# ReactiveBayes/Cortex.jl

Hardware: NVIDIA B200
Metric: message_updates_per_sec (higher is better)
Workload: dtype f32

## Files before the change

### cortex.jl_b200/csrc/grid.cu

```cuda
#include <cmath>

#include <cstring>

#include "common.cuh"

namespace cxb {

template <class T, int E>
struct VecE;
template <>
struct VecE<float, 4> {
    using type = float4;
};
template <>
struct VecE<double, 2> {
    using type = double2;
};

template <class T, int E>
__device__ __forceinline__ void load_vec(const T* p, T (&v)[E]) {
    using V = typename VecE<T, E>::type;
    V x = __ldcs(reinterpret_cast<const V*>(p));
    const T* s = reinterpret_cast<const T*>(&x);
#pragma unroll
    for (int k = 0; k < E; ++k) v[k] = s[k];
}
template <class T, int E>
__device__ __forceinline__ void store_vec(T* p, const T (&v)[E]) {
    using V = typename VecE<T, E>::type;
    V x;
    T* s = reinterpret_cast<T*>(&x);
#pragma unroll
    for (int k = 0; k < E; ++k) s[k] = v[k];
    __stcs(reinterpret_cast<V*>(p), x);
}
template <class T, int E, int LP>
__device__ __forceinline__ T group_sum(const T (&v)[E]) {
    T s = v[0];
#pragma unroll
    for (int k = 1; k < E; ++k) s += v[k];
#pragma unroll
    for (int o = LP / 2; o > 0; o >>= 1) s += __shfl_xor_sync(0xffffffffu, s, o, LP);
    return s;
}

template <class T>
__device__ __forceinline__ T rcp_pos(T x) {
    if constexpr (sizeof(T) == 4) {
        float q;
        asm("rcp.approx.ftz.f32 %0, %1;" : "=f"(q) : "f"(x));
        return fmaf(q, fmaf(-x, q, 1.0f), q);
    } else {
        return T(1) / x;
    }
}

template <class T, int E, int LP>
__device__ __forceinline__ void potts_m2v(const T (&in)[E], bool ex, T w, T (&mv)[E], bool store, void* plane, size_t o) {
    const T S = group_sum<T, E, LP>(in);
#pragma unroll
    for (int k = 0; k < E; ++k) mv[k] = S + w * in[k];
    const T tot = group_sum<T, E, LP>(mv);
    if (ex) {
        const T inv = rcp_pos<T>(tot);
#pragma unroll
        for (int k = 0; k < E; ++k) mv[k] = mv[k] * inv;
        if (store) store_vec<T, E>((T*)plane + o, mv);
    } else {
#pragma unroll
        for (int k = 0; k < E; ++k) mv[k] = T(1);
    }
}

struct GridView {
    long long H, W;
    int has_up, has_down;
    int eager_m2v;
    const void* unary;
    const void* m2f_cur[4];
    void* m2f_nxt[4];
    void* m2v[4];
    void* marg;
    const void* halo_up;
    const void* halo_down;
    void* peer_up;
    void* peer_down;
};

template <class T, int K, int E>
__global__ void __launch_bounds__(256) k_potts_sweep(GridView g, T w) {
    constexpr int LP = K / E;
    static_assert(LP >= 1 && LP <= 32 && (LP & (LP - 1)) == 0, "K / E must be a power of two <= 32");
    const long long npix = g.H * g.W;
    const long long gid = (long long)blockIdx.x * blockDim.x + threadIdx.x;
    long long pix = gid / LP;
    const int lane = (int)(gid % LP);
    const bool valid = pix < npix;
    if (!valid) pix = npix - 1;
    const long long i = pix / g.W, j = pix % g.W;
    const size_t o = (size_t)pix * K + (size_t)lane * E;

    bool ex[4];
    ex[0] = i > 0 || g.has_up;
    ex[1] = j > 0;
    ex[2] = j + 1 < g.W;
    ex[3] = i + 1 < g.H || g.has_down;

    T un[E];
    load_vec<T, E>((const T*)g.unary + o, un);

    T in[4][E];
    {
        const T* src[4];
        src[0] = (i > 0) ? (const T*)g.m2f_cur[3] + o - (size_t)g.W * K : (const T*)g.halo_up + (size_t)j * K + (size_t)lane * E;
        src[1] = (const T*)g.m2f_cur[2] + o - K;
        src[2] = (const T*)g.m2f_cur[1] + o + K;
        src[3] = (i + 1 < g.H) ? (const T*)g.m2f_cur[0] + o + (size_t)g.W * K
                               : (const T*)g.halo_down + (size_t)j * K + (size_t)lane * E;
#pragma unroll
        for (int d = 0; d < 4; ++d) {
            if (ex[d]) {
                load_vec<T, E>(src[d], in[d]);
            } else {
#pragma unroll
                for (int k = 0; k < E; ++k) in[d][k] = T(1);
            }
        }
    }
    const bool store_mv = valid && (g.eager_m2v || i == 0 || i + 1 == g.H);
    T mv[4][E];
#pragma unroll
    for (int d = 0; d < 4; ++d) {
        potts_m2v<T, E, LP>(in[d], ex[d], w, mv[d], store_mv, g.m2v[d], o);
    }
    {
        T acc[E];
#pragma unroll
        for (int k = 0; k < E; ++k) {
            T a = un[k];
            if (ex[0]) a = a * mv[0][k];
            if (ex[1]) a = a * mv[1][k];
            if (ex[2]) a = a * mv[2][k];
            if (ex[3]) a = a * mv[3][k];
            acc[k] = a;
        }
        const T inv_tot = rcp_pos<T>(group_sum<T, E, LP>(acc));
#pragma unroll
        for (int k = 0; k < E; ++k) acc[k] = acc[k] * inv_tot;
        if (valid) store_vec<T, E>((T*)g.marg + o, acc);
    }
#pragma unroll
    for (int d = 0; d < 4; ++d) {
        T acc[E];
#pragma unroll
        for (int k = 0; k < E; ++k) {
            T a = un[k];
#pragma unroll
            for (int d2 = 0; d2 < 4; ++d2)
                if (d2 != d && ex[d2]) a = a * mv[d2][k];
            acc[k] = a;
        }
        const T inv_tot = rcp_pos<T>(group_sum<T, E, LP>(acc));
#pragma unroll
        for (int k = 0; k < E; ++k) acc[k] = acc[k] * inv_tot;
        if (valid && ex[d]) store_vec<T, E>((T*)g.m2f_nxt[d] + o, acc);
        if (d == 0 && valid && i == 0 && g.peer_up) store_vec<T, E>((T*)g.peer_up + (size_t)j * K + (size_t)lane * E, acc);
        if (d == 3 && valid && i + 1 == g.H && g.peer_down) store_vec<T, E>((T*)g.peer_down + (size_t)j * K + (size_t)lane * E, acc);
    }
}

template <class T, int K, int E>
__global__ void __launch_bounds__(256) k_potts_m2v(GridView g, T w) {
    constexpr int LP = K / E;
    const long long npix = (g.H - 2) * g.W;
    const long long gid = (long long)blockIdx.x * blockDim.x + threadIdx.x;
    long long q = gid / LP;
    const int lane = (int)(gid % LP);
    const bool valid = q < npix;
    if (!valid) q = npix - 1;
    const long long pix = q + g.W;
    const long long j = pix % g.W;
    const size_t o = (size_t)pix * K + (size_t)lane * E;
    const bool ex[4] = {true, j > 0, j + 1 < g.W, true};
    const T* src[4];
    src[0] = (const T*)g.m2f_cur[3] + o - (size_t)g.W * K;
    src[1] = (const T*)g.m2f_cur[2] + o - K;
    src[2] = (const T*)g.m2f_cur[1] + o + K;
    src[3] = (const T*)g.m2f_cur[0] + o + (size_t)g.W * K;
    T in[4][E];
#pragma unroll
    for (int d = 0; d < 4; ++d) {
        if (ex[d]) {
            load_vec<T, E>(src[d], in[d]);
        } else {
#pragma unroll
            for (int k = 0; k < E; ++k) in[d][k] = T(1);
        }
    }
#pragma unroll
    for (int d = 0; d < 4; ++d) {
        T mv[E];
        potts_m2v<T, E, LP>(in[d], ex[d], w, mv, valid, g.m2v[d], o);
    }
}

__global__ void k_halo_wait(const volatile unsigned* flag_a, const volatile unsigned* flag_b, unsigned expected, unsigned long long timeout_ns,
                            unsigned* timed_out) {
    unsigned long long t0;
    asm volatile("mov.u64 %0, %%globaltimer;" : "=l"(t0));
    auto wait = [&](const volatile unsigned* f, unsigned bit) {
        while (*f < expected) {
            __nanosleep(64);
            unsigned long long t;
            asm volatile("mov.u64 %0, %%globaltimer;" : "=l"(t));
            if (t - t0 > timeout_ns) {
                atomicOr(timed_out, bit);
                return;
            }
        }
    };
    if (flag_a) wait(flag_a, 1u);
    if (flag_b) wait(flag_b, 2u);
    __threadfence_system();
}
__global__ void k_halo_signal(unsigned* peer_flag_a, unsigned* peer_flag_b, unsigned value) {
    __threadfence_system();
    if (peer_flag_a) *(volatile unsigned*)peer_flag_a = value;
    if (peer_flag_b) *(volatile unsigned*)peer_flag_b = value;
    __threadfence_system();
}

template <class T>
__global__ void k_fill(T* p, size_t n, T v) {
    size_t i = (size_t)blockIdx.x * blockDim.x + threadIdx.x;
    if (i < n) p[i] = v;
}

struct Grid {
    int device = 0, dtype = CXB_F32, K = 0, has_up = 0, has_down = 0, cur = 0;
    long long H = 0, W = 0;
    double beta = 0;
    cudaStream_t stream = nullptr;
    cudaEvent_t ev0 = nullptr, ev1 = nullptr;
    std::string err;
    DBuf<unsigned char> unary, m2f[2], m2v, marg, halo_recv;
    DBuf<unsigned> flags;
    DBuf<unsigned char> unary_alt, marg_alt;
    unsigned char *cur_unary = nullptr, *cur_marg = nullptr;
    cudaStream_t s_in = nullptr, s_out = nullptr;
    cudaEvent_t ev_in[2] = {nullptr, nullptr}, ev_sw[2] = {nullptr, nullptr}, ev_out[2] = {nullptr, nullptr};
    unsigned long long job_no = 0;
    unsigned sweep_no = 0;
    unsigned long long halo_timeout_ns = 20ull * 1000000000ull;
    bool eager_m2v = false, m2v_pending = false;
    int32_t check_halo() {
        if (!peer_halo[0] && !peer_halo[1]) return CXB_OK;
        unsigned t = 0;
        if (cudaMemcpy(&t, flags.p + 2, sizeof(unsigned), cudaMemcpyDeviceToHost) != cudaSuccess) return CXB_ERR_CUDA;
        if (!t) return CXB_OK;
        err = std::string("fused halo exchange: the row neighbour ") + ((t & 1) ? "above" : "below") +
              " did not deliver its boundary messages in time (its sweep was never enqueued, or the process is gone)";
        return CXB_ERR_STATE;
    }
    unsigned char* peer_halo[2] = {nullptr, nullptr};
    unsigned* peer_flags[2] = {nullptr, nullptr};
    void* ipc_opened[4] = {nullptr, nullptr, nullptr, nullptr};
    bool have_unary = false, have_msgs = false, ran = false;
    size_t esz() const { return dtype == CXB_F32 ? 4 : 8; }
    size_t plane() const { return (size_t)H * W * K * esz(); }
    size_t row() const { return (size_t)W * K * esz(); }
    ~Grid() {
        for (void* q : ipc_opened)
            if (q) cudaIpcCloseMemHandle(q);
        if (ev0) cudaEventDestroy(ev0);
        if (ev1) cudaEventDestroy(ev1);
        for (int i = 0; i < 2; ++i) {
            if (ev_in[i]) cudaEventDestroy(ev_in[i]);
            if (ev_sw[i]) cudaEventDestroy(ev_sw[i]);
            if (ev_out[i]) cudaEventDestroy(ev_out[i]);
        }
        if (s_in) cudaStreamDestroy(s_in);
        if (s_out) cudaStreamDestroy(s_out);
        if (stream) cudaStreamDestroy(stream);
    }
    int32_t init() {
        int count = 0;
        if (cudaGetDeviceCount(&count) != cudaSuccess || count == 0) {
            err = "no CUDA device available (cortex_b200 has no CPU fallback)";
            return CXB_ERR_CUDA;
        }
        int E = dtype == CXB_F32 ? 4 : 2;
        int LP = K / E;
        if (device < 0 || device >= count || H <= 0 || W <= 0 || K < E || K % E || LP > 32 || (LP & (LP - 1))) {
            err = "bad device / shape (labels must be 4,8,...,128 for fp32 and 2,4,...,64 for fp64, a power of two)";
            return CXB_ERR_BAD_ARG;
        }
        CXB_CUDA(cudaSetDevice(device));
        CXB_CUDA(cudaStreamCreateWithFlags(&stream, cudaStreamNonBlocking));
        if (const char* e = getenv("CXB_GRID_HALO_TIMEOUT_MS")) halo_timeout_ns = (unsigned long long)std::max(1, atoi(e)) * 1000000ull;
        if (const char* e = getenv("CXB_GRID_EAGER_M2V")) eager_m2v = atoi(e) != 0;
        CXB_CUDA(cudaEventCreate(&ev0));
        CXB_CUDA(cudaEventCreate(&ev1));
        CXB_CUDA(unary.reserve(plane()));
        CXB_CUDA(m2f[0].reserve(4 * plane()));
        CXB_CUDA(m2f[1].reserve(4 * plane()));
        CXB_CUDA(m2v.reserve(4 * plane()));
        CXB_CUDA(marg.reserve(plane()));
        CXB_CUDA(halo_recv.reserve(4 * row()));
        CXB_CUDA(flags.reserve(4));
        CXB_CUDA(cudaMemsetAsync(flags.p, 0, 4 * sizeof(unsigned), stream));
        CXB_CUDA(cudaMemsetAsync(m2v.p, 0, 4 * plane(), stream));
        CXB_CUDA(cudaMemsetAsync(marg.p, 0, plane(), stream));
        return CXB_OK;
    }
    template <class T>
    int32_t fill(void* p, size_t n, double v) {
        CXB_LAUNCH(k_fill<T>, cdiv(n, 256), 256, 0, stream, (T*)p, n, (T)v);
        return CXB_OK;
    }
    int32_t reset() {
        CXB_CUDA(cudaSetDevice(device));
        if (int32_t st = flush_m2v()) return st;
        size_t n = (size_t)4 * H * W * K, nh = (size_t)4 * W * K;
        double u = 1.0 / K;
        for (int b = 0; b < 2; ++b) dtype == CXB_F32 ? fill<float>(m2f[b].p, n, u) : fill<double>(m2f[b].p, n, u);
        dtype == CXB_F32 ? fill<float>(halo_recv.p, nh, u) : fill<double>(halo_recv.p, nh, u);
        CXB_CUDA(cudaMemsetAsync(flags.p, 0, 4 * sizeof(unsigned), stream));
        CXB_CUDA(cudaGetLastError());
        CXB_CUDA(cudaStreamSynchronize(stream));
        cur = 0;
        sweep_no = 0;
        have_msgs = true;
        return CXB_OK;
    }
    GridView view(int in) const {
        GridView g{};
        g.H = H;
        g.W = W;
        g.has_up = has_up;
        g.has_down = has_down;
        g.eager_m2v = eager_m2v;
        for (int d = 0; d < 4; ++d) {
            g.m2f_cur[d] = m2f[in].p + (size_t)d * plane();
            g.m2f_nxt[d] = m2f[in ^ 1].p + (size_t)d * plane();
            g.m2v[d] = m2v.p + (size_t)d * plane();
        }
        return g;
    }
    template <class T, int E>
    int32_t launch_k(const GridView& g, bool m2v_only) {
        const T w = (T)(std::exp(beta) - 1.0);
        long long threads = (m2v_only ? H - 2 : H) * W * (K / E);
        unsigned grid = cdiv((size_t)threads, 256);
        switch (K / E) {
#define CASE(LPV)                                                                                      \
    case LPV:                                                                                          \
        if (m2v_only)                                                                                  \
            CXB_LAUNCH((k_potts_m2v<T, LPV * E, E>), grid, 256, 0, stream, g, w);                      \
        else                                                                                           \
            CXB_LAUNCH((k_potts_sweep<T, LPV * E, E>), grid, 256, 0, stream, g, w);                    \
        break;
            CASE(1)
            CASE(2)
            CASE(4)
            CASE(8)
            CASE(16)
            CASE(32)
#undef CASE
        }
        return CXB_OK;
    }
    int32_t sweep(int64_t* n_updates) {
        if (!have_unary || !have_msgs) {
            err = "set the unary evidence and reset the messages first";
            return CXB_ERR_STATE;
        }
        CXB_CUDA(cudaSetDevice(device));
        GridView g = view(cur);
        g.unary = cur_unary ? cur_unary : unary.p;
        g.marg = cur_marg ? cur_marg : marg.p;
        const size_t par = (size_t)(sweep_no & 1) * 2 * row(), nxt_par = (size_t)((sweep_no + 1) & 1) * 2 * row();
        g.halo_up = halo_recv.p + par;
        g.halo_down = halo_recv.p + par + row();
        g.peer_up = peer_halo[0] ? peer_halo[0] + nxt_par + row() : nullptr;
        g.peer_down = peer_halo[1] ? peer_halo[1] + nxt_par : nullptr;
        const bool fused = peer_halo[0] || peer_halo[1];
        if (fused && sweep_no > 0)
            CXB_LAUNCH(k_halo_wait, 1, 1, 0, stream, peer_halo[0] ? flags.p + 0 : nullptr, peer_halo[1] ? flags.p + 1 : nullptr, sweep_no,
                       halo_timeout_ns, flags.p + 2);
        CXB_CUDA(cudaEventRecord(ev0, stream));
        int32_t st = dtype == CXB_F32 ? launch_k<float, 4>(g, false) : launch_k<double, 2>(g, false);
        if (st) return st;
        CXB_CUDA(cudaEventRecord(ev1, stream));
        m2v_pending = !eager_m2v;
        if (fused)
            CXB_LAUNCH(k_halo_signal, 1, 1, 0, stream, peer_flags[0] ? peer_flags[0] + 1 : nullptr, peer_flags[1] ? peer_flags[1] + 0 : nullptr,
                       sweep_no + 1);
        CXB_CUDA(cudaGetLastError());
        cur ^= 1;
        ++sweep_no;
        ran = true;
        if (n_updates) {
            long long vert = (H - 1) * W * 2 + (has_up ? W : 0) + (has_down ? W : 0);
            long long horz = H * (W - 1) * 2;
            *n_updates = 2 * (vert + horz) + H * W;
        }
        return CXB_OK;
    }
    int32_t flush_m2v() {
        if (!m2v_pending) return CXB_OK;
        CXB_CUDA(cudaSetDevice(device));
        if (H > 2) {
            const GridView g = view(cur ^ 1);
            int32_t st = dtype == CXB_F32 ? launch_k<float, 4>(g, true) : launch_k<double, 2>(g, true);
            if (st) return st;
            CXB_CUDA(cudaGetLastError());
        }
        m2v_pending = false;
        return CXB_OK;
    }
    int32_t infer_host(const void* unary_host, void* marg_out_host, int n_sweeps, int64_t* n_updates) {
        if (!have_msgs) {
            err = "reset the messages first";
            return CXB_ERR_STATE;
        }
        CXB_CUDA(cudaSetDevice(device));
        if (!s_in) {
            CXB_CUDA(unary_alt.reserve(plane()));
            CXB_CUDA(marg_alt.reserve(plane()));
            CXB_CUDA(cudaStreamCreateWithFlags(&s_in, cudaStreamNonBlocking));
            CXB_CUDA(cudaStreamCreateWithFlags(&s_out, cudaStreamNonBlocking));
            for (int i = 0; i < 2; ++i) {
                CXB_CUDA(cudaEventCreateWithFlags(&ev_in[i], cudaEventDisableTiming));
                CXB_CUDA(cudaEventCreateWithFlags(&ev_sw[i], cudaEventDisableTiming));
                CXB_CUDA(cudaEventCreateWithFlags(&ev_out[i], cudaEventDisableTiming));
            }
            CXB_CUDA(cudaStreamSynchronize(stream));
        }
        const int b = (int)(job_no & 1);
        unsigned char* U = b ? unary_alt.p : unary.p;
        unsigned char* M = b ? marg_alt.p : marg.p;
        if (job_no >= 2) CXB_CUDA(cudaStreamWaitEvent(s_in, ev_sw[b], 0));
        CXB_CUDA(cudaMemcpyAsync(U, unary_host, plane(), cudaMemcpyHostToDevice, s_in));
        CXB_CUDA(cudaEventRecord(ev_in[b], s_in));
        CXB_CUDA(cudaStreamWaitEvent(stream, ev_in[b], 0));
        if (job_no >= 2) CXB_CUDA(cudaStreamWaitEvent(stream, ev_out[b], 0));
        cur_unary = U;
        cur_marg = M;
        have_unary = true;
        int64_t upd = 0;
        for (int k = 0; k < n_sweeps; ++k) {
            int32_t st = sweep(&upd);
            if (st) return st;
        }
        CXB_CUDA(cudaEventRecord(ev_sw[b], stream));
        CXB_CUDA(cudaStreamWaitEvent(s_out, ev_sw[b], 0));
        CXB_CUDA(cudaMemcpyAsync(marg_out_host, M, plane(), cudaMemcpyDeviceToHost, s_out));
        CXB_CUDA(cudaEventRecord(ev_out[b], s_out));
        ++job_no;
        if (n_updates) *n_updates = upd * n_sweeps;
        return CXB_OK;
    }
    int32_t sync_all() {
        CXB_CUDA(cudaSetDevice(device));
        CXB_CUDA(cudaStreamSynchronize(stream));
        if (s_in) CXB_CUDA(cudaStreamSynchronize(s_in));
        if (s_out) CXB_CUDA(cudaStreamSynchronize(s_out));
        return check_halo();
    }
};

}

using cxb::Grid;
static inline Grid* GR(cxb_grid* g) { return reinterpret_cast<Grid*>(g); }
#define GR_CUDA(g, expr)                                        \
    do {                                                        \
        cudaError_t e__ = (expr);                               \
        if (e__ != cudaSuccess) {                               \
            GR(g)->err = ::cxb::cuda_msg(e__, #expr);           \
            return CXB_ERR_CUDA;                                \
        }                                                       \
    } while (0)

extern "C" {

int32_t cxb_grid_create(int32_t device, int32_t dtype, int64_t rows, int64_t cols, int32_t n_labels, double beta,
                        int32_t has_upper, int32_t has_lower, cxb_grid** out) try {
    if (!out || (dtype != CXB_F32 && dtype != CXB_F64)) return CXB_ERR_BAD_ARG;
    *out = nullptr;
    Grid* g = new Grid();
    g->device = device;
    g->dtype = dtype;
    g->H = rows;
    g->W = cols;
    g->K = n_labels;
    g->beta = beta;
    g->has_up = has_upper ? 1 : 0;
    g->has_down = has_lower ? 1 : 0;
    int32_t st = g->init();
    if (st) {
        fprintf(stderr, "cxb_grid_create: %s\n", g->err.c_str());
        delete g;
        return st;
    }
    *out = reinterpret_cast<cxb_grid*>(g);
    return CXB_OK;
} CXB_ABI_CATCH(CXB_ERR_INTERNAL)
void cxb_grid_destroy(cxb_grid* g) {
    if (g) {
        cudaSetDevice(GR(g)->device);
        delete GR(g);
    }
}
const char* cxb_grid_last_error(cxb_grid* g) { return g ? GR(g)->err.c_str() : "null handle"; }
int32_t cxb_grid_set_unary(cxb_grid* g, const void* unary_host) try {
    Grid* h = GR(g);
    GR_CUDA(g, cudaSetDevice(h->device));
    GR_CUDA(g, cudaMemcpyAsync(h->cur_unary ? h->cur_unary : h->unary.p, unary_host, h->plane(), cudaMemcpyHostToDevice, h->stream));
    GR_CUDA(g, cudaStreamSynchronize(h->stream));
    h->have_unary = true;
    return CXB_OK;
} CXB_ABI_CATCH(CXB_ERR_INTERNAL)
int32_t cxb_grid_reset_messages(cxb_grid* g) try { return GR(g)->reset(); } CXB_ABI_CATCH(CXB_ERR_INTERNAL)
int32_t cxb_grid_sweep(cxb_grid* g, int64_t* n_updates_out) try { return GR(g)->sweep(n_updates_out); } CXB_ABI_CATCH(CXB_ERR_INTERNAL)
void* cxb_grid_halo_send_ptr(cxb_grid* g, int32_t direction) {
    Grid* h = GR(g);
    unsigned char* base = h->m2f[h->cur].p;
    if (direction == 0) return base + 0 * h->plane();
    if (direction == 1) return base + 3 * h->plane() + (size_t)(h->H - 1) * h->row();
    return nullptr;
}
void* cxb_grid_halo_recv_ptr(cxb_grid* g, int32_t direction) {
    Grid* h = GR(g);
    unsigned char* base = h->halo_recv.p + (size_t)(h->sweep_no & 1) * 2 * h->row();
    if (direction == 0) return base;
    if (direction == 1) return base + h->row();
    return nullptr;
}
int32_t cxb_grid_p2p_export(cxb_grid* g, void* handles_out) try {
    Grid* h = GR(g);
    GR_CUDA(g, cudaSetDevice(h->device));
    cudaIpcMemHandle_t hh[2];
    GR_CUDA(g, cudaIpcGetMemHandle(&hh[0], h->halo_recv.p));
    GR_CUDA(g, cudaIpcGetMemHandle(&hh[1], h->flags.p));
    memcpy(handles_out, hh, sizeof(hh));
    return CXB_OK;
} CXB_ABI_CATCH(CXB_ERR_INTERNAL)
int32_t cxb_grid_p2p_connect_ipc(cxb_grid* g, int32_t direction, const void* neighbour_handles) try {
    Grid* h = GR(g);
    if (direction != 0 && direction != 1) return CXB_ERR_BAD_ARG;
    GR_CUDA(g, cudaSetDevice(h->device));
    cudaIpcMemHandle_t hh[2];
    memcpy(hh, neighbour_handles, sizeof(hh));
    void *halo = nullptr, *fl = nullptr;
    GR_CUDA(g, cudaIpcOpenMemHandle(&halo, hh[0], cudaIpcMemLazyEnablePeerAccess));
    GR_CUDA(g, cudaIpcOpenMemHandle(&fl, hh[1], cudaIpcMemLazyEnablePeerAccess));
    h->ipc_opened[2 * direction] = halo;
    h->ipc_opened[2 * direction + 1] = fl;
    h->peer_halo[direction] = (unsigned char*)halo;
    h->peer_flags[direction] = (unsigned*)fl;
    return CXB_OK;
} CXB_ABI_CATCH(CXB_ERR_INTERNAL)
int32_t cxb_grid_p2p_connect_local(cxb_grid* g, int32_t direction, cxb_grid* neighbour) try {
    Grid *h = GR(g), *nb = GR(neighbour);
    if ((direction != 0 && direction != 1) || !nb || nb->W != h->W || nb->K != h->K || nb->dtype != h->dtype) return CXB_ERR_BAD_ARG;
    if (nb->device != h->device) {
        int can = 0;
        GR_CUDA(g, cudaDeviceCanAccessPeer(&can, h->device, nb->device));
        if (!can) {
            h->err = "no peer access between the two devices";
            return CXB_ERR_CUDA;
        }
        GR_CUDA(g, cudaSetDevice(h->device));
        cudaError_t e = cudaDeviceEnablePeerAccess(nb->device, 0);
        if (e != cudaSuccess && e != cudaErrorPeerAccessAlreadyEnabled) GR_CUDA(g, e);
        (void)cudaGetLastError();
    }
    h->peer_halo[direction] = nb->halo_recv.p;
    h->peer_flags[direction] = nb->flags.p;
    return CXB_OK;
} CXB_ABI_CATCH(CXB_ERR_INTERNAL)
int64_t cxb_grid_halo_elems(cxb_grid* g) try { return GR(g)->W * GR(g)->K; } CXB_ABI_CATCH(-1)
int32_t cxb_grid_get_marginals(cxb_grid* g, void* out_host) try {
    Grid* h = GR(g);
    GR_CUDA(g, cudaSetDevice(h->device));
    GR_CUDA(g, cudaMemcpyAsync(out_host, h->cur_marg ? h->cur_marg : h->marg.p, h->plane(), cudaMemcpyDeviceToHost, h->stream));
    GR_CUDA(g, cudaStreamSynchronize(h->stream));
    return h->check_halo();
} CXB_ABI_CATCH(CXB_ERR_INTERNAL)
int32_t cxb_grid_get_messages(cxb_grid* g, int32_t which, void* out_host) try {
    Grid* h = GR(g);
    if (which < 0 || which > 7) {
        h->err = "message plane must be 0..7";
        return CXB_ERR_BAD_ARG;
    }
    const unsigned char* src = which < 4 ? h->m2v.p + (size_t)which * h->plane() : h->m2f[h->cur].p + (size_t)(which - 4) * h->plane();
    GR_CUDA(g, cudaSetDevice(h->device));
    if (which < 4)
        if (int32_t st = h->flush_m2v()) return st;
    GR_CUDA(g, cudaMemcpyAsync(out_host, src, h->plane(), cudaMemcpyDeviceToHost, h->stream));
    GR_CUDA(g, cudaStreamSynchronize(h->stream));
    return CXB_OK;
} CXB_ABI_CATCH(CXB_ERR_INTERNAL)
void* cxb_grid_stream(cxb_grid* g) { return (void*)GR(g)->stream; }
int32_t cxb_grid_last_kernel_ms(cxb_grid* g, float* ms_out) try {
    Grid* h = GR(g);
    if (!h->ran) {
        h->err = "no sweep has run yet";
        return CXB_ERR_STATE;
    }
    GR_CUDA(g, cudaEventSynchronize(h->ev1));
    GR_CUDA(g, cudaEventElapsedTime(ms_out, h->ev0, h->ev1));
    return CXB_OK;
} CXB_ABI_CATCH(CXB_ERR_INTERNAL)
int32_t cxb_grid_infer_host(cxb_grid* g, const void* unary_host, void* marginals_out_host, int32_t n_sweeps, int64_t* n_updates_out) try {
    return GR(g)->infer_host(unary_host, marginals_out_host, n_sweeps, n_updates_out);
} CXB_ABI_CATCH(CXB_ERR_INTERNAL)
int32_t cxb_grid_sync(cxb_grid* g) try {
    return GR(g)->sync_all();
} CXB_ABI_CATCH(CXB_ERR_INTERNAL)

}
```

Baseline: 83.52 billion.

## Fuse two Potts BP sweeps per launch with shared-memory temporal tiling

```diff
diff --git a/cortex.jl_b200/csrc/grid.cu b/cortex.jl_b200/csrc/grid.cu
--- a/cortex.jl_b200/csrc/grid.cu
+++ b/cortex.jl_b200/csrc/grid.cu
@@ -72,6 +72,48 @@
     }
 }
 
+template <class T, int E, int LP, class PutMarg, class PutM2f>
+__device__ __forceinline__ void potts_pixel(const T (&in)[4][E], const bool (&ex)[4], const T (&un)[E], T w, bool store_mv,
+                                            void* const (&m2v)[4], size_t o, PutMarg&& put_marg, PutM2f&& put_m2f) {
+    T mv[4][E];
+#pragma unroll
+    for (int d = 0; d < 4; ++d) {
+        potts_m2v<T, E, LP>(in[d], ex[d], w, mv[d], store_mv, m2v[d], o);
+    }
+    {
+        T acc[E];
+#pragma unroll
+        for (int k = 0; k < E; ++k) {
+            T a = un[k];
+            if (ex[0]) a = a * mv[0][k];
+            if (ex[1]) a = a * mv[1][k];
+            if (ex[2]) a = a * mv[2][k];
+            if (ex[3]) a = a * mv[3][k];
+            acc[k] = a;
+        }
+        const T inv_tot = rcp_pos<T>(group_sum<T, E, LP>(acc));
+#pragma unroll
+        for (int k = 0; k < E; ++k) acc[k] = acc[k] * inv_tot;
+        put_marg(acc);
+    }
+#pragma unroll
+    for (int d = 0; d < 4; ++d) {
+        T acc[E];
+#pragma unroll
+        for (int k = 0; k < E; ++k) {
+            T a = un[k];
+#pragma unroll
+            for (int d2 = 0; d2 < 4; ++d2)
+                if (d2 != d && ex[d2]) a = a * mv[d2][k];
+            acc[k] = a;
+        }
+        const T inv_tot = rcp_pos<T>(group_sum<T, E, LP>(acc));
+#pragma unroll
+        for (int k = 0; k < E; ++k) acc[k] = acc[k] * inv_tot;
+        put_m2f(d, acc);
+    }
+}
+
 struct GridView {
     long long H, W;
     int has_up, has_down;
@@ -79,6 +121,7 @@
     const void* unary;
     const void* m2f_cur[4];
     void* m2f_nxt[4];
+    void* m2f_mid[4];
     void* m2v[4];
     void* marg;
     const void* halo_up;
@@ -88,7 +131,7 @@
 };
 
 template <class T, int K, int E>
-__global__ void __launch_bounds__(256) k_potts_sweep(GridView g, T w) {
+__global__ void __launch_bounds__(256, sizeof(T) == 4 && K > 4 ? 5 : 4) k_potts_sweep(GridView g, T w) {
     constexpr int LP = K / E;
     static_assert(LP >= 1 && LP <= 32 && (LP & (LP - 1)) == 0, "K / E must be a power of two <= 32");
     const long long npix = g.H * g.W;
@@ -128,44 +171,153 @@
         }
     }
     const bool store_mv = valid && (g.eager_m2v || i == 0 || i + 1 == g.H);
-    T mv[4][E];
-#pragma unroll
-    for (int d = 0; d < 4; ++d) {
-        potts_m2v<T, E, LP>(in[d], ex[d], w, mv[d], store_mv, g.m2v[d], o);
-    }
-    {
-        T acc[E];
-#pragma unroll
-        for (int k = 0; k < E; ++k) {
-            T a = un[k];
-            if (ex[0]) a = a * mv[0][k];
-            if (ex[1]) a = a * mv[1][k];
-            if (ex[2]) a = a * mv[2][k];
-            if (ex[3]) a = a * mv[3][k];
-            acc[k] = a;
-        }
-        const T inv_tot = rcp_pos<T>(group_sum<T, E, LP>(acc));
-#pragma unroll
-        for (int k = 0; k < E; ++k) acc[k] = acc[k] * inv_tot;
-        if (valid) store_vec<T, E>((T*)g.marg + o, acc);
-    }
-#pragma unroll
-    for (int d = 0; d < 4; ++d) {
-        T acc[E];
-#pragma unroll
-        for (int k = 0; k < E; ++k) {
-            T a = un[k];
-#pragma unroll
-            for (int d2 = 0; d2 < 4; ++d2)
-                if (d2 != d && ex[d2]) a = a * mv[d2][k];
-            acc[k] = a;
-        }
-        const T inv_tot = rcp_pos<T>(group_sum<T, E, LP>(acc));
-#pragma unroll
-        for (int k = 0; k < E; ++k) acc[k] = acc[k] * inv_tot;
-        if (valid && ex[d]) store_vec<T, E>((T*)g.m2f_nxt[d] + o, acc);
-        if (d == 0 && valid && i == 0 && g.peer_up) store_vec<T, E>((T*)g.peer_up + (size_t)j * K + (size_t)lane * E, acc);
-        if (d == 3 && valid && i + 1 == g.H && g.peer_down) store_vec<T, E>((T*)g.peer_down + (size_t)j * K + (size_t)lane * E, acc);
+    potts_pixel<T, E, LP>(
+        in, ex, un, w, store_mv, g.m2v, o,
+        [&](const T(&acc)[E]) {
+            if (valid) store_vec<T, E>((T*)g.marg + o, acc);
+        },
+        [&](int d, const T(&acc)[E]) {
+            if (valid && ex[d]) store_vec<T, E>((T*)g.m2f_nxt[d] + o, acc);
+            if (d == 0 && valid && i == 0 && g.peer_up) store_vec<T, E>((T*)g.peer_up + (size_t)j * K + (size_t)lane * E, acc);
+            if (d == 3 && valid && i + 1 == g.H && g.peer_down)
+                store_vec<T, E>((T*)g.peer_down + (size_t)j * K + (size_t)lane * E, acc);
+        });
+}
+
+constexpr int FUSED_THREADS = 256;
+constexpr int FUSED_NS = 2;
+constexpr int FUSED_MAX_VEC_BYTES = 64;
+
+__device__ __forceinline__ int ring_slot(int d, long long i) {
+    return d == 0 ? 0 : d == 1 ? 1 + (int)(i & 1) : d == 2 ? 3 + (int)(i & 1) : 5 + (int)i % 3;
+}
+
+template <class T, int E>
+__device__ __forceinline__ void load_vec_l2(const T* p, T (&v)[E]) {
+    using V = typename VecE<T, E>::type;
+    V x = __ldg(reinterpret_cast<const V*>(p));
+    const T* s = reinterpret_cast<const T*>(&x);
+#pragma unroll
+    for (int k = 0; k < E; ++k) v[k] = s[k];
+}
+template <class T, int E>
+__device__ __forceinline__ void lds_vec(const T* p, T (&v)[E]) {
+    using V = typename VecE<T, E>::type;
+    V x = *reinterpret_cast<const V*>(p);
+    const T* s = reinterpret_cast<const T*>(&x);
+#pragma unroll
+    for (int k = 0; k < E; ++k) v[k] = s[k];
+}
+template <class T, int E>
+__device__ __forceinline__ void sts_vec(T* p, const T (&v)[E]) {
+    using V = typename VecE<T, E>::type;
+    V x;
+    T* s = reinterpret_cast<T*>(&x);
+#pragma unroll
+    for (int k = 0; k < E; ++k) s[k] = v[k];
+    *reinterpret_cast<V*>(p) = x;
+}
+
+template <class T, int K, int E, int NS>
+__global__ void __launch_bounds__(FUSED_THREADS, sizeof(T) == 8 ? 2 : K == 16 ? 4 : 3) k_potts_sweeps(GridView g, T w, long long BH) {
+    constexpr int LP = K / E, PX = FUSED_THREADS / LP, BW = PX - 2 * (NS - 1);
+    static_assert(NS >= 2 && BW > 0, "tile too narrow");
+    extern __shared__ __align__(16) unsigned char smem[];
+    T* ring = reinterpret_cast<T*>(smem);
+    T* unr = ring + (size_t)(NS - 1) * 8 * PX * K;
+    const long long H = g.H, W = g.W;
+    const int p = threadIdx.x / LP, lane = threadIdx.x % LP;
+    const long long r0 = (long long)blockIdx.y * BH, c0 = (long long)blockIdx.x * BW;
+    const long long x0 = c0 - (NS - 1);
+    const int xo = p * K + lane * E;
+    const long long j1 = x0 + p;
+
+    auto load_row = [&](long long i, T (&in)[4][E], T (&un)[E]) {
+        const bool valid = i < H && j1 >= 0 && j1 < W;
+        const bool ex[4] = {valid && i > 0, valid && j1 > 0, valid && j1 + 1 < W, valid && i + 1 < H};
+        const size_t o = (size_t)(valid ? i * W + j1 : 0) * K + (size_t)lane * E;
+        const T* src[4] = {(const T*)g.m2f_cur[3] + o - (size_t)W * K, (const T*)g.m2f_cur[2] + o - K,
+                           (const T*)g.m2f_cur[1] + o + K, (const T*)g.m2f_cur[0] + o + (size_t)W * K};
+#pragma unroll
+        for (int d = 0; d < 4; ++d) {
+            if (ex[d]) {
+                load_vec_l2<T, E>(src[d], in[d]);
+            } else {
+#pragma unroll
+                for (int k = 0; k < E; ++k) in[d][k] = T(1);
+            }
+        }
+        if (valid) {
+            load_vec_l2<T, E>((const T*)g.unary + o, un);
+        } else {
+#pragma unroll
+            for (int k = 0; k < E; ++k) un[k] = T(1);
+        }
+    };
+
+    const long long t_first = r0 - (NS - 1) > 0 ? r0 - (NS - 1) : 0;
+    const long long t_last = r0 + BH + NS - 2;
+    for (long long t = t_first; t <= t_last; ++t) {
+        T cin[4][E], cun[E];
+        load_row(t, cin, cun);
+#pragma unroll 1
+        for (int q = 1; q <= NS; ++q) {
+            const long long i = t - (q - 1);
+            const long long lo = r0 - (NS - q), hi = r0 + BH + (NS - q);
+            if (i >= 0 && i >= lo && i < hi && i < H) {
+                const int x = p + (q - 1);
+                const long long j = x0 + x;
+                const bool valid = x < PX - (q - 1) && j >= 0 && j < W;
+                const bool ex[4] = {valid && i > 0, valid && j > 0, valid && j + 1 < W, valid && i + 1 < H};
+                T in[4][E], un[E];
+                T* unrow = unr + (size_t)((int)i % NS) * PX * K;
+                if (q == 1) {
+#pragma unroll
+                    for (int d = 0; d < 4; ++d)
+#pragma unroll
+                        for (int k = 0; k < E; ++k) in[d][k] = cin[d][k];
+#pragma unroll
+                    for (int k = 0; k < E; ++k) un[k] = cun[k];
+                    sts_vec<T, E>(unrow + xo, un);
+                } else {
+                    const T* R = ring + (size_t)(q - 2) * 8 * PX * K;
+                    const int xk = x * K + lane * E;
+                    const T* src[4] = {R + (size_t)ring_slot(3, i - 1) * PX * K + xk, R + (size_t)ring_slot(2, i) * PX * K + xk - K,
+                                       R + (size_t)ring_slot(1, i) * PX * K + xk + K, R + (size_t)ring_slot(0, i + 1) * PX * K + xk};
+#pragma unroll
+                    for (int d = 0; d < 4; ++d) {
+                        if (ex[d]) {
+                            lds_vec<T, E>(src[d], in[d]);
+                        } else {
+#pragma unroll
+                            for (int k = 0; k < E; ++k) in[d][k] = T(1);
+                        }
+                    }
+                    if (valid) {
+                        lds_vec<T, E>(unrow + x * K + lane * E, un);
+                    } else {
+#pragma unroll
+                        for (int k = 0; k < E; ++k) un[k] = T(1);
+                    }
+                }
+                const bool owned = valid && i >= r0 && i < r0 + BH && j >= c0 && j < c0 + BW;
+                const size_t o = (size_t)(i * W + j) * K + (size_t)lane * E;
+                const bool last = q == NS;
+                T* Wr = ring + (size_t)(q - 1) * 8 * PX * K + x * K + lane * E;
+                potts_pixel<T, E, LP>(
+                    in, ex, un, w, last && owned && (i == 0 || i + 1 == H), g.m2v, o,
+                    [&](const T(&acc)[E]) {
+                        if (last && owned) store_vec<T, E>((T*)g.marg + o, acc);
+                    },
+                    [&](int d, const T(&acc)[E]) {
+                        if (!ex[d]) return;
+                        if (!last) sts_vec<T, E>(Wr + (size_t)ring_slot(d, i) * PX * K, acc);
+                        if (q == NS - 1 && owned) store_vec<T, E>((T*)g.m2f_mid[d] + o, acc);
+                        if (last && owned) store_vec<T, E>((T*)g.m2f_nxt[d] + o, acc);
+                    });
+            }
+            __syncthreads();
+        }
     }
 }
 
@@ -237,13 +389,14 @@
 }
 
 struct Grid {
-    int device = 0, dtype = CXB_F32, K = 0, has_up = 0, has_down = 0, cur = 0;
+    int device = 0, dtype = CXB_F32, K = 0, has_up = 0, has_down = 0;
+    int cur = 0, prv = 1, spare = 2;
     long long H = 0, W = 0;
     double beta = 0;
     cudaStream_t stream = nullptr;
     cudaEvent_t ev0 = nullptr, ev1 = nullptr;
     std::string err;
-    DBuf<unsigned char> unary, m2f[2], m2v, marg, halo_recv;
+    DBuf<unsigned char> unary, m2f[3], m2v, marg, halo_recv;
     DBuf<unsigned> flags;
     DBuf<unsigned char> unary_alt, marg_alt;
     unsigned char *cur_unary = nullptr, *cur_marg = nullptr;
@@ -253,6 +406,9 @@
     unsigned sweep_no = 0;
     unsigned long long halo_timeout_ns = 20ull * 1000000000ull;
     bool eager_m2v = false, m2v_pending = false;
+    int fuse_ns = 1, pending = 0;
+    int last_launch_sweeps = 1;
+    int fused_slots = 0;
     int32_t check_halo() {
         if (!peer_halo[0] && !peer_halo[1]) return CXB_OK;
         unsigned t = 0;
@@ -299,11 +455,22 @@
         CXB_CUDA(cudaStreamCreateWithFlags(&stream, cudaStreamNonBlocking));
         if (const char* e = getenv("CXB_GRID_HALO_TIMEOUT_MS")) halo_timeout_ns = (unsigned long long)std::max(1, atoi(e)) * 1000000ull;
         if (const char* e = getenv("CXB_GRID_EAGER_M2V")) eager_m2v = atoi(e) != 0;
+        int per_pass = 0;
+        if (const char* e = getenv("CXB_GRID_SWEEPS_PER_PASS")) {
+            per_pass = atoi(e);
+            if (per_pass != 1 && per_pass != FUSED_NS) {
+                err = "CXB_GRID_SWEEPS_PER_PASS must be 1 or " + std::to_string(FUSED_NS);
+                return CXB_ERR_BAD_ARG;
+            }
+        }
+        int l2 = 0;
+        CXB_CUDA(cudaDeviceGetAttribute(&l2, cudaDevAttrL2CacheSize, device));
+        const bool applies = !has_up && !has_down && !eager_m2v && K * esz() <= (size_t)FUSED_MAX_VEC_BYTES;
+        if (applies && (per_pass == FUSED_NS || (per_pass == 0 && 4 * plane() > (size_t)l2))) fuse_ns = FUSED_NS;
         CXB_CUDA(cudaEventCreate(&ev0));
         CXB_CUDA(cudaEventCreate(&ev1));
         CXB_CUDA(unary.reserve(plane()));
-        CXB_CUDA(m2f[0].reserve(4 * plane()));
-        CXB_CUDA(m2f[1].reserve(4 * plane()));
+        for (int b = 0; b < (fuse_ns > 1 ? 3 : 2); ++b) CXB_CUDA(m2f[b].reserve(4 * plane()));
         CXB_CUDA(m2v.reserve(4 * plane()));
         CXB_CUDA(marg.reserve(plane()));
         CXB_CUDA(halo_recv.reserve(4 * row()));
@@ -320,20 +487,24 @@
     }
     int32_t reset() {
         CXB_CUDA(cudaSetDevice(device));
+        if (int32_t st = flush()) return st;
         if (int32_t st = flush_m2v()) return st;
         size_t n = (size_t)4 * H * W * K, nh = (size_t)4 * W * K;
         double u = 1.0 / K;
-        for (int b = 0; b < 2; ++b) dtype == CXB_F32 ? fill<float>(m2f[b].p, n, u) : fill<double>(m2f[b].p, n, u);
+        for (auto& b : m2f)
+            if (b.p) dtype == CXB_F32 ? fill<float>(b.p, n, u) : fill<double>(b.p, n, u);
         dtype == CXB_F32 ? fill<float>(halo_recv.p, nh, u) : fill<double>(halo_recv.p, nh, u);
         CXB_CUDA(cudaMemsetAsync(flags.p, 0, 4 * sizeof(unsigned), stream));
         CXB_CUDA(cudaGetLastError());
         CXB_CUDA(cudaStreamSynchronize(stream));
         cur = 0;
+        prv = 1;
+        spare = 2;
         sweep_no = 0;
         have_msgs = true;
         return CXB_OK;
     }
-    GridView view(int in) const {
+    GridView view(int in, int out, int mid = -1) const {
         GridView g{};
         g.H = H;
         g.W = W;
@@ -342,7 +513,8 @@
         g.eager_m2v = eager_m2v;
         for (int d = 0; d < 4; ++d) {
             g.m2f_cur[d] = m2f[in].p + (size_t)d * plane();
-            g.m2f_nxt[d] = m2f[in ^ 1].p + (size_t)d * plane();
+            g.m2f_nxt[d] = m2f[out].p + (size_t)d * plane();
+            g.m2f_mid[d] = mid < 0 ? nullptr : m2f[mid].p + (size_t)d * plane();
             g.m2v[d] = m2v.p + (size_t)d * plane();
         }
         return g;
@@ -370,13 +542,81 @@
         }
         return CXB_OK;
     }
+    template <class T, int E>
+    int32_t launch_batch() {
+        constexpr int NS = FUSED_NS;
+        const T w = (T)(std::exp(beta) - 1.0);
+        GridView g = view(cur, spare, prv);
+        g.unary = cur_unary ? cur_unary : unary.p;
+        g.marg = cur_marg ? cur_marg : marg.p;
+        const int LP = K / E, PX = FUSED_THREADS / LP, BW = PX - 2 * (NS - 1);
+        const size_t smem = (size_t)(8 * (NS - 1) + NS) * FUSED_THREADS * 16;
+        const void* fn = nullptr;
+        switch (LP) {
+            case 1: fn = (const void*)k_potts_sweeps<T, 1 * E, E, NS>; break;
+            case 2: fn = (const void*)k_potts_sweeps<T, 2 * E, E, NS>; break;
+            case 4: fn = (const void*)k_potts_sweeps<T, 4 * E, E, NS>; break;
+            default: err = "k_potts_sweeps: no instance for this K"; return CXB_ERR_INTERNAL;
+        }
+        CXB_CUDA(cudaFuncSetAttribute(fn, cudaFuncAttributeMaxDynamicSharedMemorySize, (int)smem));
+        if (!fused_slots) {
+            int per_sm = 0, sms = 0;
+            CXB_CUDA(cudaOccupancyMaxActiveBlocksPerMultiprocessor(&per_sm, fn, FUSED_THREADS, smem));
+            CXB_CUDA(cudaDeviceGetAttribute(&sms, cudaDevAttrMultiProcessorCount, device));
+            fused_slots = std::max(1, per_sm * sms);
+        }
+        const long long strips = cdiv((size_t)W, (size_t)BW);
+        long long nb = std::min(std::max(1LL, fused_slots / strips), std::min(H, 65535LL));
+        const long long BH = cdiv((size_t)H, (size_t)nb);
+        nb = cdiv((size_t)H, (size_t)BH);
+        void* args[] = {&g, (void*)&w, (void*)&BH};
+        CXB_CUDA(cudaLaunchKernel(fn, dim3((unsigned)strips, (unsigned)nb), dim3(FUSED_THREADS), args, smem, stream));
+        ++g_kernel_launches;
+        return CXB_OK;
+    }
+    int32_t flush() {
+        if (!pending) return CXB_OK;
+        CXB_CUDA(cudaSetDevice(device));
+        const int n = pending;
+        pending = 0;
+        if (n == fuse_ns) {
+            CXB_CUDA(cudaEventRecord(ev0, stream));
+            int32_t st = dtype == CXB_F32 ? launch_batch<float, 4>() : launch_batch<double, 2>();
+            if (st) return st;
+            CXB_CUDA(cudaEventRecord(ev1, stream));
+            CXB_CUDA(cudaGetLastError());
+            const int c = cur;
+            cur = spare;
+            spare = c;
+            sweep_no += n;
+            last_launch_sweeps = n;
+            m2v_pending = true;
+            ran = true;
+            return CXB_OK;
+        }
+        for (int s = 0; s < n; ++s)
+            if (int32_t st = sweep_one()) return st;
+        return CXB_OK;
+    }
     int32_t sweep(int64_t* n_updates) {
         if (!have_unary || !have_msgs) {
             err = "set the unary evidence and reset the messages first";
             return CXB_ERR_STATE;
         }
+        if (n_updates) {
+            long long vert = (H - 1) * W * 2 + (has_up ? W : 0) + (has_down ? W : 0);
+            long long horz = H * (W - 1) * 2;
+            *n_updates = 2 * (vert + horz) + H * W;
+        }
+        if (fuse_ns > 1 && !peer_halo[0] && !peer_halo[1]) {
+            if (++pending == fuse_ns) return flush();
+            return CXB_OK;
+        }
+        return sweep_one();
+    }
+    int32_t sweep_one() {
         CXB_CUDA(cudaSetDevice(device));
-        GridView g = view(cur);
+        GridView g = view(cur, prv);
         g.unary = cur_unary ? cur_unary : unary.p;
         g.marg = cur_marg ? cur_marg : marg.p;
         const size_t par = (size_t)(sweep_no & 1) * 2 * row(), nxt_par = (size_t)((sweep_no + 1) & 1) * 2 * row();
@@ -397,21 +637,17 @@
             CXB_LAUNCH(k_halo_signal, 1, 1, 0, stream, peer_flags[0] ? peer_flags[0] + 1 : nullptr, peer_flags[1] ? peer_flags[1] + 0 : nullptr,
                        sweep_no + 1);
         CXB_CUDA(cudaGetLastError());
-        cur ^= 1;
+        std::swap(cur, prv);
         ++sweep_no;
+        last_launch_sweeps = 1;
         ran = true;
-        if (n_updates) {
-            long long vert = (H - 1) * W * 2 + (has_up ? W : 0) + (has_down ? W : 0);
-            long long horz = H * (W - 1) * 2;
-            *n_updates = 2 * (vert + horz) + H * W;
-        }
         return CXB_OK;
     }
     int32_t flush_m2v() {
         if (!m2v_pending) return CXB_OK;
         CXB_CUDA(cudaSetDevice(device));
         if (H > 2) {
-            const GridView g = view(cur ^ 1);
+            const GridView g = view(prv, cur);
             int32_t st = dtype == CXB_F32 ? launch_k<float, 4>(g, true) : launch_k<double, 2>(g, true);
             if (st) return st;
             CXB_CUDA(cudaGetLastError());
@@ -425,6 +661,7 @@
             return CXB_ERR_STATE;
         }
         CXB_CUDA(cudaSetDevice(device));
+        if (int32_t st = flush()) return st;
         if (!s_in) {
             CXB_CUDA(unary_alt.reserve(plane()));
             CXB_CUDA(marg_alt.reserve(plane()));
@@ -453,6 +690,7 @@
             int32_t st = sweep(&upd);
             if (st) return st;
         }
+        if (int32_t st = flush()) return st;
         CXB_CUDA(cudaEventRecord(ev_sw[b], stream));
         CXB_CUDA(cudaStreamWaitEvent(s_out, ev_sw[b], 0));
         CXB_CUDA(cudaMemcpyAsync(marg_out_host, M, plane(), cudaMemcpyDeviceToHost, s_out));
@@ -463,6 +701,7 @@
     }
     int32_t sync_all() {
         CXB_CUDA(cudaSetDevice(device));
+        if (int32_t st = flush()) return st;
         CXB_CUDA(cudaStreamSynchronize(stream));
         if (s_in) CXB_CUDA(cudaStreamSynchronize(s_in));
         if (s_out) CXB_CUDA(cudaStreamSynchronize(s_out));
@@ -517,6 +756,7 @@
 int32_t cxb_grid_set_unary(cxb_grid* g, const void* unary_host) try {
     Grid* h = GR(g);
     GR_CUDA(g, cudaSetDevice(h->device));
+    if (int32_t st = h->flush()) return st;
     GR_CUDA(g, cudaMemcpyAsync(h->cur_unary ? h->cur_unary : h->unary.p, unary_host, h->plane(), cudaMemcpyHostToDevice, h->stream));
     GR_CUDA(g, cudaStreamSynchronize(h->stream));
     h->have_unary = true;
@@ -526,6 +766,7 @@
 int32_t cxb_grid_sweep(cxb_grid* g, int64_t* n_updates_out) try { return GR(g)->sweep(n_updates_out); } CXB_ABI_CATCH(CXB_ERR_INTERNAL)
 void* cxb_grid_halo_send_ptr(cxb_grid* g, int32_t direction) {
     Grid* h = GR(g);
+    if (h->flush()) return nullptr;
     unsigned char* base = h->m2f[h->cur].p;
     if (direction == 0) return base + 0 * h->plane();
     if (direction == 1) return base + 3 * h->plane() + (size_t)(h->H - 1) * h->row();
@@ -533,6 +774,7 @@
 }
 void* cxb_grid_halo_recv_ptr(cxb_grid* g, int32_t direction) {
     Grid* h = GR(g);
+    if (h->flush()) return nullptr;
     unsigned char* base = h->halo_recv.p + (size_t)(h->sweep_no & 1) * 2 * h->row();
     if (direction == 0) return base;
     if (direction == 1) return base + h->row();
@@ -551,6 +793,7 @@
     Grid* h = GR(g);
     if (direction != 0 && direction != 1) return CXB_ERR_BAD_ARG;
     GR_CUDA(g, cudaSetDevice(h->device));
+    if (int32_t st = h->flush()) return st;
     cudaIpcMemHandle_t hh[2];
     memcpy(hh, neighbour_handles, sizeof(hh));
     void *halo = nullptr, *fl = nullptr;
@@ -565,6 +808,7 @@
 int32_t cxb_grid_p2p_connect_local(cxb_grid* g, int32_t direction, cxb_grid* neighbour) try {
     Grid *h = GR(g), *nb = GR(neighbour);
     if ((direction != 0 && direction != 1) || !nb || nb->W != h->W || nb->K != h->K || nb->dtype != h->dtype) return CXB_ERR_BAD_ARG;
+    if (int32_t st = h->flush()) return st;
     if (nb->device != h->device) {
         int can = 0;
         GR_CUDA(g, cudaDeviceCanAccessPeer(&can, h->device, nb->device));
@@ -585,6 +829,7 @@
 int32_t cxb_grid_get_marginals(cxb_grid* g, void* out_host) try {
     Grid* h = GR(g);
     GR_CUDA(g, cudaSetDevice(h->device));
+    if (int32_t st = h->flush()) return st;
     GR_CUDA(g, cudaMemcpyAsync(out_host, h->cur_marg ? h->cur_marg : h->marg.p, h->plane(), cudaMemcpyDeviceToHost, h->stream));
     GR_CUDA(g, cudaStreamSynchronize(h->stream));
     return h->check_halo();
@@ -595,8 +840,9 @@
         h->err = "message plane must be 0..7";
         return CXB_ERR_BAD_ARG;
     }
+    GR_CUDA(g, cudaSetDevice(h->device));
+    if (int32_t st = h->flush()) return st;
     const unsigned char* src = which < 4 ? h->m2v.p + (size_t)which * h->plane() : h->m2f[h->cur].p + (size_t)(which - 4) * h->plane();
-    GR_CUDA(g, cudaSetDevice(h->device));
     if (which < 4)
         if (int32_t st = h->flush_m2v()) return st;
     GR_CUDA(g, cudaMemcpyAsync(out_host, src, h->plane(), cudaMemcpyDeviceToHost, h->stream));
@@ -606,12 +852,14 @@
 void* cxb_grid_stream(cxb_grid* g) { return (void*)GR(g)->stream; }
 int32_t cxb_grid_last_kernel_ms(cxb_grid* g, float* ms_out) try {
     Grid* h = GR(g);
+    if (int32_t st = h->flush()) return st;
     if (!h->ran) {
         h->err = "no sweep has run yet";
         return CXB_ERR_STATE;
     }
     GR_CUDA(g, cudaEventSynchronize(h->ev1));
     GR_CUDA(g, cudaEventElapsedTime(ms_out, h->ev0, h->ev1));
+    *ms_out /= (float)h->last_launch_sweeps;
     return CXB_OK;
 } CXB_ABI_CATCH(CXB_ERR_INTERNAL)
 int32_t cxb_grid_infer_host(cxb_grid* g, const void* unary_host, void* marginals_out_host, int32_t n_sweeps, int64_t* n_updates_out) try {
diff --git a/profiles/time_potts_fused.py b/profiles/time_potts_fused.py
--- /dev/null
+++ b/profiles/time_potts_fused.py
@@ -0,0 +1,82 @@
+import gc
+import os
+import statistics
+import subprocess
+import sys
+
+import numpy as np
+import torch
+
+sys.path.insert(0, os.path.dirname(os.path.dirname(os.path.abspath(__file__))))
+from __graft_entry__ import load_package
+
+C = load_package()
+N = int(sys.argv[1]) if len(sys.argv) > 1 else 8192
+ROUNDS = int(sys.argv[2]) if len(sys.argv) > 2 else 3
+BATCHED = sys.argv[3] if len(sys.argv) > 3 else "default"
+K, BETA, SWEEPS = 16, 0.7, 50
+NS, THREADS, PER_SM = 2, 256, 4
+
+print(subprocess.run(["nvidia-smi", "--query-gpu=name,power.limit,clocks.max.sm", "--format=csv"], capture_output=True,
+                     text=True).stdout.strip(), flush=True)
+rng = np.random.Generator(np.random.PCG64(1234))
+unary = np.empty((N, N, K), dtype=np.float32)
+for i in range(0, N, 256):
+    e = rng.standard_exponential((min(256, N - i), N, K), dtype=np.float32)
+    unary[i:i + 256] = e / e.sum(axis=-1, keepdims=True)
+
+PX = THREADS // 4
+BW = PX - 2 * (NS - 1)
+sms = torch.cuda.get_device_properties(0).multi_processor_count
+strips = -(-N // BW)
+nb = min(max(1, PER_SM * sms // strips), N, 65535)
+BH = -(-N // nb)
+overlap = PX / BW * (BH + 2 * (NS - 1)) / BH
+bytes_single = 640
+bytes_batched = (320 * overlap + 576) / NS
+print(f"{N}^2, K = {K}: tile {BW} x {BH} (+ halo), {strips} x {-(-N // BH)} CTAs; model: single {bytes_single} B, batched "
+      f"{bytes_batched:.0f} B per pixel per sweep (read overlap {overlap:.3f})", flush=True)
+
+
+def arm(per_pass):
+    if per_pass is None:
+        os.environ.pop("CXB_GRID_SWEEPS_PER_PASS", None)
+    else:
+        os.environ["CXB_GRID_SWEEPS_PER_PASS"] = str(per_pass)
+    g = C.PottsGrid(N, N, K, BETA, dtype=C.capi.F32)
+    g.set_unary(unary)
+    g.reset_messages()
+    ext = torch.cuda.ExternalStream(g.stream)
+    for _ in range(3 * SWEEPS):
+        g.sweep()
+    g.sync()
+    l0 = C.default_api().kernel_launches()
+    e0, e1 = torch.cuda.Event(enable_timing=True), torch.cuda.Event(enable_timing=True)
+    e0.record(ext)
+    for _ in range(SWEEPS):
+        g.sweep()
+    e1.record(ext)
+    e1.synchronize()
+    launches = C.default_api().kernel_launches() - l0
+    ms = e0.elapsed_time(e1) / SWEEPS
+    del g
+    gc.collect()
+    return ms, launches
+
+
+arms = [1, None if BATCHED == "default" else int(BATCHED)]
+res = {a: [] for a in arms}
+for r in range(ROUNDS):
+    for a in arms:
+        ms, launches = arm(a)
+        res[a].append(ms)
+        name = "single (=1)" if a == 1 else f"batched ({BATCHED})"
+        print(f"round {r} {name:14s}: {ms:.3f} ms per sweep (events, {SWEEPS} sweeps in {launches} launches)", flush=True)
+for a in arms:
+    ev = res[a]
+    mean = statistics.mean(ev)
+    b = bytes_single if a == 1 else bytes_batched
+    print(f"{'single' if a == 1 else 'batched':7s}: {mean:.3f} ms per sweep, spread {min(ev):.3f} .. {max(ev):.3f} "
+          f"({(max(ev) - min(ev)) / mean * 100:.2f} %); model {b * N * N / 1e9:.2f} GB per sweep = {b * N * N / (mean * 1e6):.0f} GB/s")
+ratio = [x / y for x, y in zip(res[arms[0]], res[arms[1]])]
+print(f"single / batched per sweep: {statistics.mean(ratio):.3f} (rounds: {', '.join(f'{x:.3f}' for x in ratio)})")
```

After: 91.12 billion, median of 6. 1.09x the previous value.
